# olFi95/image_search

Measured on AMD Instinct MI355X. Metric: images/sec embedded (ViT-L/14 b=256) + queries/sec cosine top-10 over 10M x 768, higher is better.
Workload: dtype bf16; 1 GPU; BASELINE config 4: per step, H2D of a pinned batch of 256 224x224x3 f32 images -> bf16 ViT-L/14 (random-init seeded weights) -> 256 rows appended to the table on the device -> cosine top-10 query over 10000000+ x 768 fp32 rows per GPU -> D2H of the k results; fused on HIP streams (the upload runs under the previous batch's tower; the scan is asynchronous to the host and runs between towers); query; batch=256, rows_per_gpu=10000000, k=10

## Files before the change

### image_search_amd/_lib.py

```python
from __future__ import annotations

import ctypes
import os

_PKG = os.path.dirname(os.path.abspath(__file__))
LIB_PATH = os.path.join(_PKG, "libmi355clip.so")

c_f = ctypes.POINTER(ctypes.c_float)
c_u64p = ctypes.POINTER(ctypes.c_uint64)
c_u8p = ctypes.POINTER(ctypes.c_uint8)
c_vp = ctypes.c_void_p

SYMBOLS = {
    "mi_last_error": (ctypes.c_char_p, []),
    "mi_abi_version": (ctypes.c_int, []),
    "mi_device_count": (ctypes.c_int, []),
    "mi_clip_load": (ctypes.c_int, [ctypes.c_char_p, ctypes.c_int, ctypes.c_int, ctypes.POINTER(c_vp)]),
    "mi_clip_free": (None, [c_vp]),
    "mi_weights_list": (ctypes.c_int, [ctypes.c_char_p, ctypes.c_char_p, ctypes.c_size_t, ctypes.POINTER(ctypes.c_size_t)]),
    "mi_clip_set_option": (ctypes.c_int, [c_vp, ctypes.c_char_p, ctypes.c_int]),
    "mi_clip_info": (ctypes.c_int, [c_vp, ctypes.POINTER(ctypes.c_uint32)]),
    "mi_clip_ln_fold_stats": (ctypes.c_int, [c_vp, ctypes.POINTER(ctypes.c_uint64), ctypes.c_int]),
    "mi_clip_embed": (ctypes.c_int, [c_vp, c_vp, ctypes.c_size_t, c_vp]),
    "mi_clip_embed_device": (ctypes.c_int, [c_vp, c_vp, ctypes.c_size_t, c_vp, c_vp]),
# ... 91 lines not shown
    "mi_pipeline_drain": (ctypes.c_int, [c_vp, ctypes.c_uint32]),
    "mi_pipeline_stats": (ctypes.c_int, [c_vp, ctypes.POINTER(ctypes.c_double), ctypes.c_int]),
    "mi_host_alloc": (ctypes.c_int, [ctypes.c_size_t, ctypes.POINTER(c_vp)]),
    "mi_host_free": (None, [c_vp]),
    "mi_average_slices": (ctypes.c_int, [ctypes.POINTER(c_f), ctypes.c_size_t, ctypes.c_size_t, c_f]),
    "mi_refine": (ctypes.c_int, [c_f, ctypes.POINTER(c_f), ctypes.c_size_t, ctypes.c_size_t, c_f]),
    "mi_op_linear": (ctypes.c_int, [ctypes.c_int, ctypes.c_int, ctypes.c_int, c_vp, c_vp, c_vp, c_vp,
                                    ctypes.c_size_t, ctypes.c_int, ctypes.c_int]),
    "mi_op_attention": (ctypes.c_int, [ctypes.c_int, ctypes.c_int, c_vp, c_vp, ctypes.c_size_t, ctypes.c_int,
                                       ctypes.c_int, ctypes.c_int]),
    "mi_op_clock_probe": (ctypes.c_int, [ctypes.c_int, c_vp, ctypes.POINTER(ctypes.c_float)]),
    "mi_op_linear_lnf": (ctypes.c_int, [ctypes.c_int, ctypes.c_int, c_vp, c_vp, c_vp, c_vp, c_vp, c_vp,
                                        ctypes.c_size_t, ctypes.c_int, ctypes.c_int]),
    "mi_op_linear_resid24": (ctypes.c_int, [ctypes.c_int, c_vp, c_vp, c_vp, c_vp, c_vp, c_vp, c_vp,
                                            ctypes.c_size_t, ctypes.c_int, ctypes.c_int, ctypes.c_float]),
    "mi_op_layernorm": (ctypes.c_int, [ctypes.c_int, ctypes.c_int, c_vp, c_vp, c_vp, c_vp, ctypes.c_size_t,
                                       ctypes.c_int, ctypes.c_float]),
}

MI_OK = 0
ERR_NAMES = {-1: "MI_ERR_INVALID", -2: "MI_ERR_IO", -3: "MI_ERR_HIP", -4: "MI_ERR_NO_DEVICE",
             -5: "MI_ERR_UNSUPPORTED", -6: "MI_ERR_OOM"}


class MiError(RuntimeError):
    def __init__(self, code: int, msg: str):
        super().__init__(f"{ERR_NAMES.get(code, code)}: {msg}")
        self.code = code


# ... 27 lines not shown
```

### image_search_amd/csrc/handles.h

```cpp
#pragma once
#include <mutex>
#include <vector>

#include "common.h"

namespace mi {
typedef unsigned short bf16_t;

struct Layer {
    float *ln1w, *ln1b, *ln2w, *ln2b;
    void *wqkv, *wo, *w1, *w2;
    float *bqkv, *bo, *b1, *b2;
    void *wqkv_f = nullptr, *w1_f = nullptr;
    float *cqkv = nullptr, *bqkv_f = nullptr, *c1 = nullptr, *b1_f = nullptr;
};


}

struct mi_clip {
    int device = 0, precision = 0;
    int image = 0, patch = 0, grid = 0, S = 0, D = 0, L = 0, H = 0, FF = 0, E = 0, Kp = 0;
    float eps = 1e-5f;
    std::vector<void*> allocs;
// ... 6 lines not shown
    float *d_in = nullptr, *d_in2 = nullptr, *d_out = nullptr, *d_out2 = nullptr;
    struct Act {
        float *patch = nullptr, *x = nullptr;
        void *col = nullptr, *y = nullptr, *qkv = nullptr, *h = nullptr;
        mi::bf16_t *delta = nullptr, *delta2 = nullptr;
        void *c_ctx = nullptr, *c_y = nullptr, *c_h = nullptr;
        float* c_x = nullptr;
        mi::bf16_t *c_d1 = nullptr, *c_d2 = nullptr;
        float *part = nullptr, *stats = nullptr;
        float* c_stats = nullptr;
    } act[4];
    hipStream_t aux[3] = {nullptr, nullptr, nullptr};
    hipEvent_t ev_fork = nullptr, ev_join[3] = {nullptr, nullptr, nullptr};
    hipEvent_t ev_embed[4] = {nullptr, nullptr, nullptr, nullptr}, ev_front[4] = {nullptr, nullptr, nullptr, nullptr};
    bool ev_embed_set[4] = {false, false, false, false};
    bool x24 = true;
    bool ln_fold = true;
    bool fold_ready = false;
    bool ln_center = true;
    unsigned long long* d_fold_offset_rows = nullptr;
    uint64_t fold_rows_checked = 0;
    int parts = 2;
    int n_cu = 256;
    uint8_t* d_rgb = nullptr;
    bool text = false;
    int vocab = 0;
    float* tok = nullptr;
    int *d_ids = nullptr, *d_rows = nullptr;
    size_t text_cap = 0;
    int* h_ids_pin = nullptr;
// ... 2 lines not shown
    hipGraph_t text_graph = nullptr;
    hipGraphExec_t text_graph_exec = nullptr;
    uint8_t* d_img_src[2] = {nullptr, nullptr};
    float* d_img_tmp = nullptr;
    size_t img_src_cap = 0, img_tmp_cap = 0;
    hipStream_t copy_stream = nullptr;
    hipEvent_t ev_up[2] = {nullptr, nullptr}, ev_used[2] = {nullptr, nullptr};
    hipStream_t stream = nullptr;
    size_t max_batch = 256;
    bool split_ln = false;
    int attn_ver = 2;
    bool q_prescaled = false;
    bool attn_shift = false;
    int qkv_pad = 128;
    int qkv_layout = 0;
    bool front_overlap = false;
    bool store_nt = true;
    bool attn_nt = false;
    int attn_order = 1;
    bool full_last = false;
    bool split_tail = true;
    int gemm_order = 4;
    bool text_fast = true;
    bool attn_f32_mfma = true;
    bool text_fuse = true;
    int ln_nt = 0;
    bool im2col_rows = true;
    mi::WorkOrder order;
    std::mutex mu;
};

// ... 145 lines not shown
```

### image_search_amd/csrc/vit.hip

```cpp
#include <algorithm>
#include <cctype>
#include <cmath>
#include <cstdio>
#include <cstring>
#include <map>
#include <mutex>
#include <string>
#include <vector>

#include "common.h"
#include "handles.h"
#include "weights.h"
#include "../../include/mi355clip_ops.h"
#include "preprocess_kernels.h"
#include "vit_kernels.h"
#include "attn32_kernels.h"

using namespace mi;

namespace {

inline uint16_t f32_to_bf16_host(float f) {
    uint32_t u;
    std::memcpy(&u, &f, 4);
    if ((u & 0x7fffffffu) > 0x7f800000u) return (uint16_t)((u >> 16) | 0x40);
    return (uint16_t)((u + 0x7fffu + ((u >> 16) & 1u)) >> 16);
}

}

namespace {
// ... 383 lines not shown
        return;
    }
    if constexpr (EPI == EPI_BIAS || EPI == EPI_BIAS_QGELU) {
        const size_t Mp = pad256(Mrows);
        if (m->precision == MI_PRECISION_BF16 && pp_shape_ok(Mp, N, K, col_stride == 64 ? ldo : N)) {
            PpFold f;
            f.col_stride = col_stride;
            launch_pp<EPI>(m, X, W, bias, out, Mp, N, K, ldo, f, s);
            return;
        }
    }
    if (col_stride != 64) fail(MI_ERR_INVALID, "head-major output needs the persistent GEMM");
    gemm_p<EPI>(m->precision, X, W, bias, out, Mrows, N, K, ldo, s);
}

#define MI_LN_DISPATCH(D, CALL)                                                              \
    switch (D) {                                                                             \
        case 128: { constexpr int VEC = 2, NT = 1; CALL; } break;                            \
        case 256: { constexpr int VEC = 4, NT = 1; CALL; } break;                            \
        case 384: { constexpr int VEC = 2, NT = 3; CALL; } break;                            \
        case 512: { constexpr int VEC = 4, NT = 2; CALL; } break;                            \
        case 768: { constexpr int VEC = 4, NT = 3; CALL; } break;                            \
        case 1024: { constexpr int VEC = 4, NT = 4; CALL; } break;                           \
        case 1280: { constexpr int VEC = 4, NT = 5; CALL; } break;                           \
        case 1536: { constexpr int VEC = 4, NT = 6; CALL; } break;                           \
        case 1664: { constexpr int VEC = 2, NT = 13; CALL; } break;                          \
        default: fail(MI_ERR_UNSUPPORTED, "hidden size %d has no LayerNorm instantiation", D); \
    }

void layer_norm(mi_clip* m, float* x, const bf16_t* d1, const bf16_t* d2, bool write_back, void* y, const float* w,
// ... 139 lines not shown
        first += np;
    }
    if (parts > 1) {
        HIP_CHECK(hipEventRecord(m->ev_fork, s0));
        for (int p = 1; p < parts; ++p) HIP_CHECK(hipStreamWaitEvent(pt[p].s, m->ev_fork, 0));
    }
    for (int p = 0; p < parts; ++p) {
        Part& q = pt[p];
        hipStream_t es_ = q.s;
        hipStream_t fs = front ? front : q.s;
        if (!m->ev_embed[p]) {
            HIP_CHECK(hipEventCreateWithFlags(&m->ev_embed[p], hipEventDisableTiming));
            HIP_CHECK(hipEventCreateWithFlags(&m->ev_front[p], hipEventDisableTiming));
        }
        if (front && m->ev_embed_set[p]) HIP_CHECK(hipStreamWaitEvent(front, m->ev_embed[p], 0));
        const size_t total = q.P * 3 * (size_t)m->patch;
        const unsigned blocks = (unsigned)std::min<size_t>((total + 255) / 256, 65535 * 4);
        if (m->precision == MI_PRECISION_F32 || is_x3(m))
            hipLaunchKernelGGL((im2col_kernel<float>), dim3(blocks), dim3(256), 0, fs, q.img, (float*)q.a->col, (int)q.n, m->grid, m->patch, m->image, m->Kp);
        else if (m->im2col_rows && m->image % 4 == 0 && (3 * m->patch * m->patch) % 4 == 0 && m->Kp % 4 == 0 && (size_t)3 * m->patch * m->image * 4 <= 64 * 1024)
            hipLaunchKernelGGL(im2col_rows_kernel, dim3((unsigned)(q.n * m->grid)), dim3(256), (size_t)3 * m->patch * m->image * 4, fs, q.img,
                               (bf16_t*)q.a->col, m->grid, m->patch, m->image, m->Kp);
        else
            hipLaunchKernelGGL((im2col_kernel<bf16_t>), dim3(blocks), dim3(256), 0, fs, q.img, (bf16_t*)q.a->col, (int)q.n, m->grid, m->patch, m->image, m->Kp);
        HIP_CHECK(hipGetLastError());
        gemm<EPI_STORE_F32>(m, q.a->col, m->wpatch, nullptr, q.a->patch, q.P, D, m->Kp, D, fs);
        if (front) {
            HIP_CHECK(hipEventRecord(m->ev_front[p], front));
            HIP_CHECK(hipStreamWaitEvent(es_, m->ev_front[p], 0));
        }
        fs = es_;
        const size_t rows_launch = fold ? pad256(q.M) : q.M;
        const unsigned lb = (unsigned)((rows_launch + 3) / 4);
        MI_LN_DISPATCH(D, hipLaunchKernelGGL((embed_ln_kernel<VEC, NT>), dim3(lb), dim3(256), 0, fs, q.a->patch, m->cls, m->pos, q.a->x, m->pre_w, m->pre_b, (int)q.M, S, m->eps, q.xlo,
                                             fold ? q.a->stats : (float*)nullptr, (int)rows_launch, fold ? m->d_fold_offset_rows : nullptr, m->ln_center ? 1 : 0));
        if (fold) m->fold_rows_checked += q.M;
        HIP_CHECK(hipEventRecord(m->ev_embed[p], fs));
        m->ev_embed_set[p] = true;
        HIP_CHECK(hipGetLastError());
    }
    const bool full_last = m->full_last;
    const int nb = D / 32;
    const int ldq = (int)qkv_pitch(m);
    const bool hm = qkv_head_major(m) && pp_shape_ok(pad256((n / parts + 1) * (size_t)S), 3 * D, D, 3 * D);
    auto hm_rows = [&](const Part& q) { return hm ? pad256(q.M) : (size_t)0; };
    auto qkv_cs = [&](const Part& q) { return hm ? (uint32_t)(pad256(q.M) * 64) : 64u; };
    const int ldq_o = hm ? 64 : ldq;
    auto ln_stats = [&](Part& q) {
        const size_t Mp = pad256(q.M);
        hipLaunchKernelGGL(ln_stats_kernel, dim3((unsigned)(Mp / 16)), dim3(256), 0, q.s, q.a->part, q.a->stats, (int)Mp, nb, 1.0f / (float)D, m->eps,
                           (int)q.M, m->d_fold_offset_rows);
        HIP_CHECK(hipGetLastError());
        m->fold_rows_checked += q.M;
    };
    for (size_t li = 0; li < m->layers.size(); ++li) {
        const Layer& ly = m->layers[li];
        const bool last = !full_last && li + 1 == m->layers.size();
// ... 20 lines not shown
                PpFold f;
                f.xlo = (uint8_t*)q.a->x + q.xlo; f.part = q.a->part;
                launch_pp<EPI_RESID24>(m, q.a->y, ly.wo, ly.bo, q.a->x, pad256(q.M), D, D, D, f, s);
                ln_stats(q);
                PpFold f1;
                f1.cvec = ly.c1; f1.stats = q.a->stats;
                launch_pp<EPI_LNF_QGELU>(m, q.a->x, ly.w1_f, ly.b1_f, q.a->h, pad256(q.M), FF, D, FF, f1, s);
                launch_pp<EPI_RESID24>(m, q.a->h, ly.w2, ly.b2, q.a->x, pad256(q.M), D, FF, D, f, s);
                ln_stats(q);
                continue;
            }
            if (last) {
                const size_t es = esize(m);
                const unsigned gb = (unsigned)std::min<size_t>((q.n * (size_t)D / 4 + 255) / 256, 4096);
                char* kv_out = (char*)q.a->qkv + (hm ? (size_t)m->H * pad256(q.M) * 64 : (size_t)D) * es;
                if (fold) {
                    PpFold f;
                    f.cvec = ly.cqkv + D; f.stats = q.a->stats; f.col_stride = qkv_cs(q);
                    launch_pp<EPI_LNF>(m, q.a->x, (const char*)ly.wqkv_f + (size_t)D * D * 2, ly.bqkv_f + D, kv_out, pad256(q.M), 2 * D, D, ldq_o, f, s);
                    hipLaunchKernelGGL((gather_rows_kernel<bf16_t>), dim3(gb), dim3(256), 0, s, (const bf16_t*)q.a->x, (bf16_t*)q.a->c_y, (int)q.n, (size_t)S, D);
                    hipLaunchKernelGGL(gather_stats_kernel, dim3((unsigned)((q.n + 255) / 256)), dim3(256), 0, s, q.a->stats, q.a->c_stats, (int)q.n, (size_t)S);
                    PpFold fq;
                    fq.cvec = ly.cqkv; fq.stats = q.a->c_stats;
                    launch_pp<EPI_LNF>(m, q.a->c_y, ly.wqkv_f, ly.bqkv_f, q.a->c_ctx, pad256(q.n), D, D, D, fq, s);
                } else {
                gemm<EPI_BIAS>(m, q.a->y, (const char*)ly.wqkv + (size_t)D * Kln * es, ly.bqkv + D, kv_out, q.M, 2 * D, Kln, ldq_o, s, qkv_cs(q));
                if (deferred) hipLaunchKernelGGL((gather_rows_kernel<bf16_t>), dim3(gb), dim3(256), 0, s, (const bf16_t*)q.a->y, (bf16_t*)q.a->c_y, (int)q.n, (size_t)S, Kln);
                else hipLaunchKernelGGL((gather_rows_kernel<float>), dim3(gb), dim3(256), 0, s, (const float*)q.a->y, (float*)q.a->c_y, (int)q.n, (size_t)S, D);
                gemm<EPI_BIAS>(m, q.a->c_y, ly.wqkv, ly.bqkv, q.a->c_ctx, q.n, D, Kln, D, s);
                }
                if (deferred) hipLaunchKernelGGL((scatter_rows_kernel<bf16_t>), dim3(gb), dim3(256), 0, s, (const bf16_t*)q.a->c_ctx, (bf16_t*)q.a->qkv, (int)q.n, (size_t)S, D, (size_t)ldq_o, (size_t)qkv_cs(q));
                else hipLaunchKernelGGL((scatter_rows_kernel<float>), dim3(gb), dim3(256), 0, s, (const float*)q.a->c_ctx, (float*)q.a->qkv, (int)q.n, (size_t)S, D, (size_t)ldq, (size_t)64);
                HIP_CHECK(hipGetLastError());
                attention(m, q.a->qkv, q.a->y, q.n, s, true, ldq, hm_rows(q));
                const unsigned gb2 = gb;
                if (deferred) hipLaunchKernelGGL((gather_rows_kernel<bf16_t>), dim3(gb2), dim3(256), 0, s, (const bf16_t*)q.a->y, (bf16_t*)q.a->c_ctx, (int)q.n, (size_t)S, D);
                else hipLaunchKernelGGL((gather_rows_kernel<float>), dim3(gb2), dim3(256), 0, s, (const float*)q.a->y, (float*)q.a->c_ctx, (int)q.n, (size_t)S, D);
                if (q.xlo) hipLaunchKernelGGL(gather_rows_x24_kernel, dim3(gb2), dim3(256), 0, s, (const uint16_t*)q.a->x, (const uint8_t*)q.a->x + q.xlo, q.a->c_x, (int)q.n, (size_t)S, D, x_bias);
                else hipLaunchKernelGGL((gather_rows_kernel<float>), dim3(gb2), dim3(256), 0, s, (const float*)q.a->x, q.a->c_x, (int)q.n, (size_t)S, D);
                HIP_CHECK(hipGetLastError());
                if (deferred) {
                    gemm<EPI_BIAS>(m, q.a->c_ctx, ly.wo, ly.bo, q.a->c_d1, q.n, D, D, D, s);
                    layer_norm(m, q.a->c_x, q.a->c_d1, nullptr, false, q.a->c_y, ly.ln2w, ly.ln2b, q.n, s);
                    gemm<EPI_BIAS_QGELU>(m, q.a->c_y, ly.w1, ly.b1, q.a->c_h, q.n, FF, Kln, FF, s);
                    gemm<EPI_BIAS>(m, q.a->c_h, ly.w2, ly.b2, q.a->c_d2, q.n, D, FF, D, s);
                } else {
                    gemm<EPI_BIAS_RESID>(m, q.a->c_ctx, ly.wo, ly.bo, q.a->c_x, q.n, D, D, D, s);
                    layer_norm(m, q.a->c_x, nullptr, nullptr, true, q.a->c_y, ly.ln2w, ly.ln2b, q.n, s);
                    gemm<EPI_BIAS_QGELU>(m, q.a->c_y, ly.w1, ly.b1, q.a->c_h, q.n, FF, Kln, FF, s);
// ... 180 lines not shown
        }
    }
    MI_LN_DISPATCH(D, hipLaunchKernelGGL((head_kernel<VEC, NT>), dim3((unsigned)((n + 7) / 8), 16), dim3(256), 0, s, a.x, p1, p2, m->post_w, m->post_b, m->proj, m->d_out, (int)n, S, m->E, m->eps, (const int*)m->d_rows));
    HIP_CHECK(hipGetLastError());
}

void free_model(mi_clip* m) {
    if (!m) return;
    (void)hipSetDevice(m->device);
    if (m->stream) { (void)hipStreamSynchronize(m->stream); (void)hipStreamDestroy(m->stream); }
    for (auto& a : m->aux) if (a) { (void)hipStreamSynchronize(a); (void)hipStreamDestroy(a); }
    m->order.destroy();
    if (m->ev_fork) (void)hipEventDestroy(m->ev_fork);
    for (auto& e : m->ev_embed) if (e) (void)hipEventDestroy(e);
    for (auto& e : m->ev_front) if (e) (void)hipEventDestroy(e);
    for (auto& e : m->ev_join) if (e) (void)hipEventDestroy(e);
    if (m->copy_stream) { (void)hipStreamSynchronize(m->copy_stream); (void)hipStreamDestroy(m->copy_stream); }
    for (int b = 0; b < 2; ++b) {
        if (m->ev_up[b]) (void)hipEventDestroy(m->ev_up[b]);
        if (m->ev_used[b]) (void)hipEventDestroy(m->ev_used[b]);
        if (m->d_img_src[b]) (void)hipFree(m->d_img_src[b]);
    }
    if (m->d_img_tmp) (void)hipFree(m->d_img_tmp);
    drop_text_graph(m);
    if (m->h_ids_pin) (void)hipHostFree(m->h_ids_pin);
    if (m->h_out_pin) (void)hipHostFree(m->h_out_pin);
    for (void* p : m->allocs) (void)hipFree(p);
    for (void* p : m->ws) (void)hipFree(p);
    delete m;
}
// ... 18 lines not shown
            const TensorInfo& t = file->info(name);
            out += name + " " + t.dtype + " [";
            for (size_t i = 0; i < t.shape.size(); ++i) out += (i ? "," : "") + std::to_string(t.shape[i]);
            out += "]\n";
        }
        for (const std::string& l : file->skipped_lines()) out += l + "\n";
        if (needed) *needed = out.size() + 1;
        if (buf && cap) {
            const size_t n = std::min(cap - 1, out.size());
            std::memcpy(buf, out.data(), n);
            buf[n] = '\0';
        }
    });
}

int mi_clip_set_option(mi_clip* m, const char* key, int value) {
    return guarded([&] {
        if (!m || !key) fail(MI_ERR_INVALID, "null argument");
        std::lock_guard<std::mutex> l(m->mu);
        DeviceGuard g(m->device);
        const std::string k(key);
        if (m->text) { m->order.sync(); drop_text_graph(m); }
        if (k == "full_last") m->full_last = value != 0;
        else if (k == "attn_shift") m->attn_shift = value != 0;
        else if (k == "front_overlap") m->front_overlap = value != 0;
        else if (k == "attn_nt") m->attn_nt = value != 0;
        else if (k == "store_nt") m->store_nt = value != 0;
        else if (k == "qkv_pad") {
            if (value < 0 || value > 1024 || value % 64) fail(MI_ERR_INVALID, "qkv_pad must be a multiple of 64 in 0..1024");
            if (m->text) fail(MI_ERR_INVALID, "the text tower's qkv rows are dense");
            if (value != m->qkv_pad) {
                m->order.sync();
                for (void* p : m->ws) HIP_CHECK(hipFree(p));
                m->ws.clear();
                m->cap = 0;
                m->qkv_pad = value;
            }
        } else if (k == "qkv_layout") {
            if (value < 0 || value > 1) fail(MI_ERR_INVALID, "qkv_layout must be 0 (token rows) or 1 (head-major planes)");
            if (m->text) fail(MI_ERR_INVALID, "the text tower's qkv rows are dense");
// ... 23 lines not shown
            m->ln_fold = value != 0;
        }
        else if (k == "max_batch") {
            if (value < 1) fail(MI_ERR_INVALID, "max_batch must be >= 1");
            m->max_batch = (size_t)value;
        } else if (k == "parts") {
            if (value < 1 || value > 4) fail(MI_ERR_INVALID, "parts must be 1..4");
            if (m->text) fail(MI_ERR_INVALID, "the text tower runs as one stream");
            if (value != m->parts) {
                m->order.sync();
                for (void* p : m->ws) HIP_CHECK(hipFree(p));
                m->ws.clear();
                m->cap = 0;
                m->parts = value;
            }
        } else fail(MI_ERR_INVALID, "unknown option '%s' (full_last, front_overlap, attn_shift, attn_nt, store_nt, attn_order, qkv_pad, qkv_layout, split_tail, gemm_order, im2col_rows, ln_nt, x24, ln_fold, text_fast, text_fuse, attn_f32_mfma, max_batch, parts)", key);
    });
}

int mi_clip_load(const char* weights_path, int device, int precision, mi_clip** out) {
    mi_clip* m = nullptr;
    const int rc = guarded([&] {
        if (!out) fail(MI_ERR_INVALID, "out is null");
        *out = nullptr;
        if (!weights_path) fail(MI_ERR_INVALID, "weights_path is null");
        if (precision != MI_PRECISION_F32 && precision != MI_PRECISION_BF16 && precision != MI_PRECISION_BF16_SPLIT &&
            precision != MI_PRECISION_BF16X3)
            fail(MI_ERR_INVALID, "precision %d: use MI_PRECISION_F32 (0), MI_PRECISION_BF16 (1), MI_PRECISION_BF16_SPLIT (2) or MI_PRECISION_BF16X3 (3)", precision);
        DeviceGuard g(device);
        m = new mi_clip();
        m->device = device;
// ... 1 lines not shown
        m->split_ln = precision == MI_PRECISION_BF16_SPLIT;
        if (const char* e = std::getenv("MI_CLIP_MAX_BATCH")) m->max_batch = std::max(1, std::atoi(e));
        HIP_CHECK(hipEventCreateWithFlags(&m->ev_fork, hipEventDisableTiming));
        for (auto& e : m->ev_join) HIP_CHECK(hipEventCreateWithFlags(&e, hipEventDisableTiming));
        if (const char* e = std::getenv("MI_CLIP_PARTS")) m->parts = std::min(4, std::max(1, std::atoi(e)));
        if (const char* e = std::getenv("MI_CLIP_FULL_LAST")) m->full_last = std::atoi(e) != 0;
        if (const char* e = std::getenv("MI_CLIP_ATTN")) m->attn_ver = std::atoi(e) == 1 ? 1 : 2;
        if (const char* e = std::getenv("MI_GEMM_SPLIT")) m->split_tail = std::atoi(e) != 0;
        if (const char* e = std::getenv("MI_GEMM_ORDER")) m->gemm_order = std::max(0, std::min(16, std::atoi(e)));
        if (const char* e = std::getenv("MI_CLIP_IM2COL")) m->im2col_rows = std::atoi(e) != 0;
        if (const char* e = std::getenv("MI_CLIP_LN_NT")) m->ln_nt = std::atoi(e) & 3;
        if (const char* e = std::getenv("MI_CLIP_X24")) m->x24 = std::atoi(e) != 0;
        if (m->precision == MI_PRECISION_BF16X3) m->x24 = false;
        if (const char* e = std::getenv("MI_CLIP_LN_CENTER")) m->ln_center = std::atoi(e) != 0;
        if (const char* e = std::getenv("MI_CLIP_QKV_LAYOUT")) m->qkv_layout = std::atoi(e) == 1 ? 1 : 0;
        if (const char* e = std::getenv("MI_CLIP_FRONT_OVERLAP")) m->front_overlap = std::atoi(e) != 0;
        hipDeviceProp_t prop;
        HIP_CHECK(hipGetDeviceProperties(&prop, device));
        m->n_cu = prop.multiProcessorCount;
        load_weights(m, weights_path);
        if (const char* e = std::getenv("MI_CLIP_LN_FOLD")) m->ln_fold = std::atoi(e) != 0 && m->fold_ready;
        *out = m;
    });
    if (rc != MI_OK && m) free_model(m);
    return rc;
}

void mi_clip_free(mi_clip* m) { free_model(m); }

int mi_clip_load_text(const char* weights_path, int device, int precision, mi_clip** out) {
    mi_clip* m = nullptr;
// ... 361 lines not shown
        void* dw = sc.up(MI_PRECISION_BF16, w, n, k, n);
        float* db = (float*)sc.up(MI_PRECISION_F32, bias, 1, n, 1);
        PpFold f;
        f.cvec = (float*)sc.up(MI_PRECISION_F32, c, 1, n, 1);
        f.stats = (float*)sc.up(MI_PRECISION_F32, stats, m_rows, 2, mp);
        void* dout = sc.bytes(mp * n * 2);
        mi_clip mm;
        op_pp_model(mm, device);
        if (epilogue == EPI_LNF) launch_pp<EPI_LNF>(&mm, dx, dw, db, dout, mp, n, k, n, f, nullptr);
        else launch_pp<EPI_LNF_QGELU>(&mm, dx, dw, db, dout, mp, n, k, n, f, nullptr);
        HIP_CHECK(hipDeviceSynchronize());
        sc.down(MI_PRECISION_BF16, dout, out, m_rows * n);
    });
}

int mi_op_linear_resid24(int device, const float* x, const float* w, const float* bias, float* xres, float* hi_out,
                         float* part, float* stats, size_t m_rows, int n, int k, float eps) {
    return guarded([&] {
        if (!x || !w || !bias || !xres) fail(MI_ERR_INVALID, "null buffer");
        const size_t mp = pad256(m_rows);
        if (!pp_shape_ok(mp, n, k, n) || mp * (size_t)(n / 32) * 8 >= (1ull << 32))
            fail(MI_ERR_UNSUPPORTED, "shape [%zu x %d x %d] is not one of the persistent GEMM's", m_rows, n, k);
        DeviceGuard g(device);
        Scratch sc;
        void* dx = sc.up(MI_PRECISION_BF16, x, m_rows, k, mp);
        void* dw = sc.up(MI_PRECISION_BF16, w, n, k, n);
        float* db = (float*)sc.up(MI_PRECISION_F32, bias, 1, n, 1);
        const size_t cnt = mp * (size_t)n;
        std::vector<uint16_t> hi(cnt, 0);
        std::vector<uint8_t> lo(cnt, 0x80);
// ... 119 lines not shown
```

### image_search_amd/ops.py

```python
from __future__ import annotations

import numpy as np

from ._lib import check, lib

EPI_STORE_F32, EPI_BIAS, EPI_BIAS_QGELU, EPI_BIAS_RESID = 0, 1, 2, 3
EPI_LNF, EPI_LNF_QGELU = 4, 5


def _f(a):
    return np.ascontiguousarray(a, np.float32)


def linear(x, w, bias=None, epilogue=EPI_BIAS, precision=0, out=None, device=0):
    x, w = _f(x), _f(w)
    m, k = x.shape
    n = w.shape[0]
    o = _f(out).copy() if out is not None else np.zeros((m, n), np.float32)
    b = _f(bias) if bias is not None else None
    check(lib().mi_op_linear(device, precision, epilogue, x.ctypes.data, w.ctypes.data,
                             b.ctypes.data if b is not None else None, o.ctypes.data, m, n, k))
    return o


# ... 22 lines not shown
                                 stats.ctypes.data, o.ctypes.data, m, n, k))
    return o


def linear_resid24(x, w, bias, xres, eps=1e-5, device=0):
    x, w, bias = _f(x), _f(w), _f(bias)
    r = _f(xres).copy()
    m, k = x.shape
    n = w.shape[0]
    hi = np.zeros((m, n), np.float32)
    part = np.zeros((m, n // 32, 2), np.float32)
    stats = np.zeros((m, 2), np.float32)
    check(lib().mi_op_linear_resid24(device, x.ctypes.data, w.ctypes.data, bias.ctypes.data, r.ctypes.data,
                                     hi.ctypes.data, part.ctypes.data, stats.ctypes.data, m, n, k, eps))
    return r, hi, part, stats
```

### include/mi355clip.h

```cpp
#ifndef MI355CLIP_H
#define MI355CLIP_H

#include <stddef.h>
#include <stdint.h>

#ifdef __cplusplus
extern "C" {
#endif

#define MI_OK 0
#define MI_ERR_INVALID (-1)
#define MI_ERR_IO (-2)
#define MI_ERR_HIP (-3)
#define MI_ERR_NO_DEVICE (-4)
#define MI_ERR_UNSUPPORTED (-5)
#define MI_ERR_OOM (-6)

#define MI_PRECISION_F32 0
#define MI_PRECISION_BF16 1
#define MI_PRECISION_BF16_SPLIT 2
#define MI_PRECISION_BF16X3 3

#define MI_KNN_NO_ID UINT64_MAX

// ... 1 lines not shown
typedef struct mi_knn mi_knn;
typedef struct mi_pipeline mi_pipeline;
typedef struct mi_knn_sharded mi_knn_sharded;
typedef struct mi_index mi_index;

const char* mi_last_error(void);
int mi_abi_version(void);
int mi_device_count(void);


int mi_clip_load(const char* weights_path, int device, int precision, mi_clip** out);
void mi_clip_free(mi_clip* m);
int mi_weights_list(const char* weights_path, char* buf, size_t cap, size_t* needed);

int mi_clip_set_option(mi_clip* m, const char* key, int value);

int mi_clip_info(const mi_clip* m, uint32_t out[8]);

int mi_clip_ln_fold_stats(mi_clip* m, uint64_t out[2], int reset);

int mi_clip_embed(mi_clip* m, const float* nchw, size_t n, float* out);

int mi_clip_embed_device(mi_clip* m, const float* d_nchw, size_t n, float* d_out, void* stream);

int mi_clip_embed_rgb8(mi_clip* m, const uint8_t* rgb8, size_t n, float* out);

int mi_preprocess_rgb8(const uint8_t* rgb8, size_t n, uint32_t height, uint32_t width, float* chw);

int mi_resize_catmullrom_rgb8(int device, const uint8_t* rgb8, uint32_t width, uint32_t height, uint32_t new_width,
                              uint32_t new_height, uint8_t* out);
// ... 120 lines not shown
```

### include/mi355clip_ops.h

```cpp
#ifndef MI355CLIP_OPS_H
#define MI355CLIP_OPS_H
#include <stddef.h>
#include <stdint.h>
#ifdef __cplusplus
extern "C" {
#endif

#define MI_EPI_STORE_F32 0
#define MI_EPI_BIAS 1
#define MI_EPI_BIAS_QGELU 2
#define MI_EPI_BIAS_RESID 3

int mi_op_linear(int device, int precision, int epilogue, const float* x, const float* w, const float* bias,
                 float* out, size_t m_rows, int n, int k);

#define MI_EPI_LNF 4
#define MI_EPI_LNF_QGELU 5
int mi_op_linear_lnf(int device, int epilogue, const float* x, const float* w, const float* bias, const float* c,
                     const float* stats, float* out, size_t m_rows, int n, int k);
int mi_op_linear_resid24(int device, const float* x, const float* w, const float* bias, float* xres, float* hi_out,
                         float* part, float* stats, size_t m_rows, int n, int k, float eps);

int mi_op_attention(int device, int precision, const float* qkv, float* ctx, size_t n_img, int s_tok, int d,
                    int heads);

int mi_op_layernorm(int device, int precision, const float* x, const float* w, const float* b, float* y,
                    size_t rows, int d, float eps);

int mi_op_clock_probe(int device, void* stream, float* mhz);

#ifdef __cplusplus
}
#endif
#endif
```

Baseline: 6628 images/s.

## Add dedicated CLS-row tail kernels for the last layer and overlap next front

Adds a CLS tail path, on by default, for the deferred last layer. Only the CLS rows get their Q projection, out-projection, LN2 and MLP, through a small MFMA GEMM kernel that reads strided CLS rows directly, which removes the gather and scatter kernels and the generic GEMM launches that are inefficient at tiny M. A fused LN2 kernel reads the packed residual in place. A new front_overlap=2 mode lets the next batch's front end wait only on the tail event after attention rather than on the full embed. It also adds option validation and a test entry point. The cost is more code paths, and the new GEMM streams weights without LDS reuse.

```diff
diff --git a/image_search_amd/_lib.py b/image_search_amd/_lib.py
--- a/image_search_amd/_lib.py
+++ b/image_search_amd/_lib.py
@@ -129,6 +129,9 @@
                                         ctypes.c_size_t, ctypes.c_int, ctypes.c_int]),
     "mi_op_linear_resid24": (ctypes.c_int, [ctypes.c_int, c_vp, c_vp, c_vp, c_vp, c_vp, c_vp, c_vp,
                                             ctypes.c_size_t, ctypes.c_int, ctypes.c_int, ctypes.c_float]),
+    "mi_clip_option_check": (ctypes.c_int, [ctypes.c_char_p, ctypes.c_int]),
+    "mi_op_linear_cls": (ctypes.c_int, [ctypes.c_int, ctypes.c_int, c_vp, c_vp, c_vp, c_vp, c_vp, c_vp,
+                                        ctypes.c_size_t, ctypes.c_int, ctypes.c_int, ctypes.c_size_t, ctypes.c_int]),
     "mi_op_layernorm": (ctypes.c_int, [ctypes.c_int, ctypes.c_int, c_vp, c_vp, c_vp, c_vp, ctypes.c_size_t,
                                        ctypes.c_int, ctypes.c_float]),
 }
diff --git a/image_search_amd/csrc/cls_tail_kernels.h b/image_search_amd/csrc/cls_tail_kernels.h
--- /dev/null
+++ b/image_search_amd/csrc/cls_tail_kernels.h
@@ -0,0 +1,95 @@
+#pragma once
+#include "vit_kernels.h"
+
+namespace mi {
+
+constexpr int CLS_ROWS = 64;
+
+template <int EPI, int P>
+__global__ __launch_bounds__(256) void cls_gemm_kernel(const bf16_t* __restrict__ X, size_t ldx, const bf16_t* __restrict__ W, int K,
+                                                       const float* __restrict__ bias, const float* __restrict__ cvec,
+                                                       const float* __restrict__ stats, size_t ld_stats, bf16_t* __restrict__ out,
+                                                       size_t ldo, uint32_t cs, int M) {
+    static_assert(EPI == EPI_BIAS || EPI == EPI_BIAS_QGELU || EPI == EPI_LNF, "the tail's three epilogues");
+    const int lane = threadIdx.x & 63, wave = threadIdx.x >> 6, g = lane >> 4, l15 = lane & 15;
+    const int n0 = blockIdx.x * 16;
+    const int m0 = blockIdx.y * CLS_ROWS + wave * 16;
+    if (m0 >= M) return;
+    const int row = min(m0 + l15, M - 1);
+    const bf16_t* wp = W + (size_t)(n0 + l15) * K + 8 * g;
+    const bf16_t* xp = X + (size_t)row * ldx + 8 * g;
+    bf16x8 a[P], b[P];
+#pragma unroll
+    for (int i = 0; i < P; ++i) {
+        a[i] = *reinterpret_cast<const bf16x8*>(wp + 32 * i);
+        b[i] = *reinterpret_cast<const bf16x8*>(xp + 32 * i);
+    }
+    const v4f b4 = *reinterpret_cast<const v4f*>(bias + n0 + 4 * g);
+    v4f c4 = (v4f){0.0f, 0.0f, 0.0f, 0.0f};
+    v2f st = (v2f){0.0f, 0.0f};
+    if constexpr (EPI == EPI_LNF) {
+        c4 = *reinterpret_cast<const v4f*>(cvec + n0 + 4 * g);
+        st = *reinterpret_cast<const v2f*>(stats + (size_t)row * ld_stats * 2);
+    }
+    v4f acc = (v4f){0.0f, 0.0f, 0.0f, 0.0f};
+    const int steps = K / 32;
+    for (int k = P; k < steps; k += P) {
+#pragma unroll
+        for (int i = 0; i < P; ++i) {
+            acc = __builtin_amdgcn_mfma_f32_16x16x32_bf16(a[i], b[i], acc, 0, 0, 0);
+            a[i] = *reinterpret_cast<const bf16x8*>(wp + 32 * (k + i));
+            b[i] = *reinterpret_cast<const bf16x8*>(xp + 32 * (k + i));
+        }
+    }
+#pragma unroll
+    for (int i = 0; i < P; ++i) acc = __builtin_amdgcn_mfma_f32_16x16x32_bf16(a[i], b[i], acc, 0, 0, 0);
+    v4f v;
+    if constexpr (EPI == EPI_LNF) {
+#pragma unroll
+        for (int c = 0; c < 4; ++c) v[c] = __builtin_fmaf(st.x, acc[c], __builtin_fmaf(st.y, c4[c], b4[c]));
+    } else {
+        v = acc + b4;
+    }
+    if constexpr (EPI == EPI_BIAS_QGELU) {
+#pragma unroll
+        for (int c = 0; c < 4; ++c) v[c] = quick_gelu<true>(v[c]);
+    }
+    if (m0 + l15 >= M) return;
+    const int col = n0 + 4 * g;
+    v2u pk;
+    pk.x = pack2bf(v[0], v[1]);
+    pk.y = pack2bf(v[2], v[3]);
+    *reinterpret_cast<v2u*>(out + (size_t)row * ldo + (size_t)(col >> 6) * cs + (col & 63)) = pk;
+}
+
+template <int VEC, int NT>
+__global__ __launch_bounds__(256) void cls_ln2_kernel(const float* __restrict__ x, size_t x_lo_off, uint32_t x_bias, size_t S,
+                                                      const bf16_t* __restrict__ d1, float* __restrict__ cx, bf16_t* __restrict__ y,
+                                                      const float* __restrict__ w, const float* __restrict__ b, int rows, float eps,
+                                                      int y_ld, int split) {
+    constexpr int D = 64 * VEC * NT;
+    const int lane = threadIdx.x & 63;
+    const int row = blockIdx.x * 4 + (threadIdx.x >> 6);
+    if (row >= rows) return;
+    const size_t src = (size_t)row * S * D;
+    LnRow<VEC, NT> r;
+    bool packed = false;
+    if constexpr (VEC == 4) {
+        if (x_lo_off) {
+            r.load_x24(reinterpret_cast<const uint16_t*>(x) + src, reinterpret_cast<const uint8_t*>(x) + x_lo_off + src, lane, x_bias);
+            packed = true;
+        }
+    }
+    if (!packed) r.load(x + src, lane);
+    r.store(cx + (size_t)row * D, lane);
+    r.add_bf16(d1 + (size_t)row * D, lane);
+    r.normalize(w, b, eps, lane);
+    r.store(y + (size_t)row * y_ld, lane);
+    if (split) {
+#pragma unroll
+        for (int j = 0; j < VEC * NT; ++j) r.v[j] -= bf2f(f2bf(r.v[j]));
+        r.store(y + (size_t)row * y_ld + D, lane);
+    }
+}
+
+}
diff --git a/image_search_amd/csrc/handles.h b/image_search_amd/csrc/handles.h
--- a/image_search_amd/csrc/handles.h
+++ b/image_search_amd/csrc/handles.h
@@ -44,6 +44,8 @@
     hipEvent_t ev_fork = nullptr, ev_join[3] = {nullptr, nullptr, nullptr};
     hipEvent_t ev_embed[4] = {nullptr, nullptr, nullptr, nullptr}, ev_front[4] = {nullptr, nullptr, nullptr, nullptr};
     bool ev_embed_set[4] = {false, false, false, false};
+    hipEvent_t ev_tail[4] = {nullptr, nullptr, nullptr, nullptr};
+    bool ev_tail_set[4] = {false, false, false, false};
     bool x24 = true;
     bool ln_fold = true;
     bool fold_ready = false;
@@ -76,7 +78,8 @@
     bool attn_shift = false;
     int qkv_pad = 128;
     int qkv_layout = 0;
-    bool front_overlap = false;
+    bool cls_tail = true;
+    int front_overlap = 0;
     bool store_nt = true;
     bool attn_nt = false;
     int attn_order = 1;
diff --git a/image_search_amd/csrc/vit.hip b/image_search_amd/csrc/vit.hip
--- a/image_search_amd/csrc/vit.hip
+++ b/image_search_amd/csrc/vit.hip
@@ -15,6 +15,7 @@
 #include "preprocess_kernels.h"
 #include "vit_kernels.h"
 #include "attn32_kernels.h"
+#include "cls_tail_kernels.h"
 
 using namespace mi;
 
@@ -428,6 +429,22 @@
     gemm_p<EPI>(m->precision, X, W, bias, out, Mrows, N, K, ldo, s);
 }
 
+bool cls_gemm_shape_ok(int N, int K) { return N % 16 == 0 && K % 256 == 0; }
+template <int EPI>
+void launch_cls_gemm(const void* X, size_t ldx, const void* W, const float* bias, const float* cvec, const float* stats, size_t ld_stats,
+                     void* out, size_t ldo, uint32_t cs, size_t M, int N, int K, hipStream_t s) {
+    if (M == 0) return;
+    if (!cls_gemm_shape_ok(N, K)) fail(MI_ERR_UNSUPPORTED, "CLS GEMM: N=%d must be a multiple of 16 and K=%d of 256", N, K);
+    const dim3 grid((unsigned)(N / 16), (unsigned)((M + CLS_ROWS - 1) / CLS_ROWS));
+    if (K % 512 == 0)
+        hipLaunchKernelGGL((cls_gemm_kernel<EPI, 16>), grid, dim3(256), 0, s, (const bf16_t*)X, ldx, (const bf16_t*)W, K, bias, cvec, stats, ld_stats,
+                           (bf16_t*)out, ldo, cs, (int)M);
+    else
+        hipLaunchKernelGGL((cls_gemm_kernel<EPI, 8>), grid, dim3(256), 0, s, (const bf16_t*)X, ldx, (const bf16_t*)W, K, bias, cvec, stats, ld_stats,
+                           (bf16_t*)out, ldo, cs, (int)M);
+    HIP_CHECK(hipGetLastError());
+}
+
 #define MI_LN_DISPATCH(D, CALL)                                                              \
     switch (D) {                                                                             \
         case 128: { constexpr int VEC = 2, NT = 1; CALL; } break;                            \
@@ -597,6 +614,9 @@
             HIP_CHECK(hipEventCreateWithFlags(&m->ev_front[p], hipEventDisableTiming));
         }
         if (front && m->ev_embed_set[p]) HIP_CHECK(hipStreamWaitEvent(front, m->ev_embed[p], 0));
+        if (front && p == 0 && m->front_overlap == 2)
+            for (int t = 0; t < 4; ++t)
+                if (m->ev_tail_set[t]) HIP_CHECK(hipStreamWaitEvent(front, m->ev_tail[t], 0));
         const size_t total = q.P * 3 * (size_t)m->patch;
         const unsigned blocks = (unsigned)std::min<size_t>((total + 255) / 256, 65535 * 4);
         if (m->precision == MI_PRECISION_F32 || is_x3(m))
@@ -624,6 +644,10 @@
     }
     const bool full_last = m->full_last;
     const int nb = D / 32;
+    const size_t np_max = pad256(n / parts + 1);
+    const bool cls_tail = m->cls_tail && deferred && cls_gemm_shape_ok(D, fold ? D : Kln) && cls_gemm_shape_ok(D, D) &&
+                          cls_gemm_shape_ok(FF, Kln) && cls_gemm_shape_ok(D, FF) && pp_shape_ok(np_max, D, fold ? D : Kln, D) &&
+                          pp_shape_ok(np_max, D, D, D) && pp_shape_ok(np_max, FF, Kln, FF) && pp_shape_ok(np_max, D, FF, D);
     const int ldq = (int)qkv_pitch(m);
     const bool hm = qkv_head_major(m) && pp_shape_ok(pad256((n / parts + 1) * (size_t)S), 3 * D, D, 3 * D);
     auto hm_rows = [&](const Part& q) { return hm ? pad256(q.M) : (size_t)0; };
@@ -674,6 +698,33 @@
                 const size_t es = esize(m);
                 const unsigned gb = (unsigned)std::min<size_t>((q.n * (size_t)D / 4 + 255) / 256, 4096);
                 char* kv_out = (char*)q.a->qkv + (hm ? (size_t)m->H * pad256(q.M) * 64 : (size_t)D) * es;
+                if (cls_tail) {
+                    const size_t ldo_q = (size_t)S * ldq_o;
+                    if (fold) {
+                        launch_cls_gemm<EPI_LNF>(q.a->x, (size_t)S * D, ly.wqkv_f, ly.bqkv_f, ly.cqkv, q.a->stats, (size_t)S, q.a->qkv, ldo_q, qkv_cs(q),
+                                                 q.n, D, D, s);
+                        PpFold f;
+                        f.cvec = ly.cqkv + D; f.stats = q.a->stats; f.col_stride = qkv_cs(q);
+                        launch_pp<EPI_LNF>(m, q.a->x, (const char*)ly.wqkv_f + (size_t)D * D * 2, ly.bqkv_f + D, kv_out, pad256(q.M), 2 * D, D, ldq_o, f, s);
+                    } else {
+                        launch_cls_gemm<EPI_BIAS>(q.a->y, (size_t)S * Kln, ly.wqkv, ly.bqkv, nullptr, nullptr, 0, q.a->qkv, ldo_q, qkv_cs(q), q.n, D, Kln, s);
+                        gemm<EPI_BIAS>(m, q.a->y, (const char*)ly.wqkv + (size_t)D * Kln * es, ly.bqkv + D, kv_out, q.M, 2 * D, Kln, ldq_o, s, qkv_cs(q));
+                    }
+                    attention(m, q.a->qkv, q.a->y, q.n, s, true, ldq, hm_rows(q));
+                    if (!m->ev_tail[p]) HIP_CHECK(hipEventCreateWithFlags(&m->ev_tail[p], hipEventDisableTiming));
+                    HIP_CHECK(hipEventRecord(m->ev_tail[p], s));
+                    m->ev_tail_set[p] = true;
+                    launch_cls_gemm<EPI_BIAS>(q.a->y, (size_t)S * D, ly.wo, ly.bo, nullptr, nullptr, 0, q.a->c_d1, D, 64, q.n, D, D, s);
+                    MI_LN_DISPATCH(D, hipLaunchKernelGGL((cls_ln2_kernel<VEC, NT>), dim3((unsigned)((q.n + 3) / 4)), dim3(256), 0, s, q.a->x, q.xlo, x_bias, (size_t)S,
+                                                         q.a->c_d1, q.a->c_x, (bf16_t*)q.a->c_y, ly.ln2w, ly.ln2b, (int)q.n, m->eps, Kln, m->split_ln ? 1 : 0));
+                    HIP_CHECK(hipGetLastError());
+                    launch_cls_gemm<EPI_BIAS_QGELU>(q.a->c_y, Kln, ly.w1, ly.b1, nullptr, nullptr, 0, q.a->c_h, FF, 64, q.n, FF, Kln, s);
+                    launch_cls_gemm<EPI_BIAS>(q.a->c_h, FF, ly.w2, ly.b2, nullptr, nullptr, 0, q.a->c_d2, D, 64, q.n, D, FF, s);
+                    const unsigned hy = (unsigned)std::max(16, std::min(64, m->E / 16));
+                    MI_LN_DISPATCH(D, hipLaunchKernelGGL((head_kernel<VEC, NT>), dim3((unsigned)((q.n + 7) / 8), hy), dim3(256), 0, s, q.a->c_x, q.a->c_d1, q.a->c_d2, m->post_w, m->post_b, m->proj, q.out, (int)q.n, 1, m->E, m->eps, (const int*)nullptr));
+                    HIP_CHECK(hipGetLastError());
+                    continue;
+                }
                 if (fold) {
                     PpFold f;
                     f.cvec = ly.cqkv + D; f.stats = q.a->stats; f.col_stride = qkv_cs(q);
@@ -693,6 +744,9 @@
                 else hipLaunchKernelGGL((scatter_rows_kernel<float>), dim3(gb), dim3(256), 0, s, (const float*)q.a->c_ctx, (float*)q.a->qkv, (int)q.n, (size_t)S, D, (size_t)ldq, (size_t)64);
                 HIP_CHECK(hipGetLastError());
                 attention(m, q.a->qkv, q.a->y, q.n, s, true, ldq, hm_rows(q));
+                if (!m->ev_tail[p]) HIP_CHECK(hipEventCreateWithFlags(&m->ev_tail[p], hipEventDisableTiming));
+                HIP_CHECK(hipEventRecord(m->ev_tail[p], s));
+                m->ev_tail_set[p] = true;
                 const unsigned gb2 = gb;
                 if (deferred) hipLaunchKernelGGL((gather_rows_kernel<bf16_t>), dim3(gb2), dim3(256), 0, s, (const bf16_t*)q.a->y, (bf16_t*)q.a->c_ctx, (int)q.n, (size_t)S, D);
                 else hipLaunchKernelGGL((gather_rows_kernel<float>), dim3(gb2), dim3(256), 0, s, (const float*)q.a->y, (float*)q.a->c_ctx, (int)q.n, (size_t)S, D);
@@ -903,6 +957,7 @@
     if (m->ev_fork) (void)hipEventDestroy(m->ev_fork);
     for (auto& e : m->ev_embed) if (e) (void)hipEventDestroy(e);
     for (auto& e : m->ev_front) if (e) (void)hipEventDestroy(e);
+    for (auto& e : m->ev_tail) if (e) (void)hipEventDestroy(e);
     for (auto& e : m->ev_join) if (e) (void)hipEventDestroy(e);
     if (m->copy_stream) { (void)hipStreamSynchronize(m->copy_stream); (void)hipStreamDestroy(m->copy_stream); }
     for (int b = 0; b < 2; ++b) {
@@ -951,16 +1006,61 @@
     });
 }
 
+namespace {
+struct OptionSpec { const char* key; int lo, hi; const char* bounds; };
+constexpr int OPT_MIN = -2147483647 - 1, OPT_MAX = 2147483647;
+const OptionSpec kOptions[] = {
+    {"full_last", OPT_MIN, OPT_MAX, ""},
+    {"front_overlap", 0, 2, "front_overlap must be 0 (off), 1 (behind the upload) or 2 (under the previous forward's CLS tail)"},
+    {"cls_tail", OPT_MIN, OPT_MAX, ""},
+    {"attn_shift", OPT_MIN, OPT_MAX, ""},
+    {"attn_nt", OPT_MIN, OPT_MAX, ""},
+    {"store_nt", OPT_MIN, OPT_MAX, ""},
+    {"attn_order", 0, 1, "attn_order must be 0 or 1"},
+    {"qkv_pad", 0, 1024, "qkv_pad must be a multiple of 64 in 0..1024"},
+    {"qkv_layout", 0, 1, "qkv_layout must be 0 (token rows) or 1 (head-major planes)"},
+    {"split_tail", OPT_MIN, OPT_MAX, ""},
+    {"gemm_order", 0, 16, "gemm_order must be 0..16"},
+    {"im2col_rows", OPT_MIN, OPT_MAX, ""},
+    {"ln_nt", OPT_MIN, OPT_MAX, ""},
+    {"x24", OPT_MIN, OPT_MAX, ""},
+    {"ln_fold", OPT_MIN, OPT_MAX, ""},
+    {"text_fast", OPT_MIN, OPT_MAX, ""},
+    {"text_fuse", OPT_MIN, OPT_MAX, ""},
+    {"attn_f32_mfma", OPT_MIN, OPT_MAX, ""},
+    {"max_batch", 1, OPT_MAX, "max_batch must be >= 1"},
+    {"parts", 1, 4, "parts must be 1..4"},
+};
+void option_check(const char* key, int value) {
+    if (!key) fail(MI_ERR_INVALID, "null argument");
+    std::string names;
+    for (const OptionSpec& o : kOptions) {
+        if (std::strcmp(o.key, key) == 0) {
+            if (value < o.lo || value > o.hi) fail(MI_ERR_INVALID, "%s", o.bounds);
+            return;
+        }
+        names += (names.empty() ? "" : ", ") + std::string(o.key);
+    }
+    fail(MI_ERR_INVALID, "unknown option '%s' (%s)", key, names.c_str());
+}
+}
+
+int mi_clip_option_check(const char* key, int value) {
+    return guarded([&] { option_check(key, value); });
+}
+
 int mi_clip_set_option(mi_clip* m, const char* key, int value) {
     return guarded([&] {
         if (!m || !key) fail(MI_ERR_INVALID, "null argument");
+        option_check(key, value);
         std::lock_guard<std::mutex> l(m->mu);
         DeviceGuard g(m->device);
         const std::string k(key);
         if (m->text) { m->order.sync(); drop_text_graph(m); }
         if (k == "full_last") m->full_last = value != 0;
         else if (k == "attn_shift") m->attn_shift = value != 0;
-        else if (k == "front_overlap") m->front_overlap = value != 0;
+        else if (k == "front_overlap") m->front_overlap = value;
+        else if (k == "cls_tail") m->cls_tail = value != 0;
         else if (k == "attn_nt") m->attn_nt = value != 0;
         else if (k == "store_nt") m->store_nt = value != 0;
         else if (k == "qkv_pad") {
@@ -1014,7 +1114,7 @@
                 m->cap = 0;
                 m->parts = value;
             }
-        } else fail(MI_ERR_INVALID, "unknown option '%s' (full_last, front_overlap, attn_shift, attn_nt, store_nt, attn_order, qkv_pad, qkv_layout, split_tail, gemm_order, im2col_rows, ln_nt, x24, ln_fold, text_fast, text_fuse, attn_f32_mfma, max_batch, parts)", key);
+        } else fail(MI_ERR_INVALID, "option '%s' is listed but not handled", key);
     });
 }
 
@@ -1046,7 +1146,8 @@
         if (m->precision == MI_PRECISION_BF16X3) m->x24 = false;
         if (const char* e = std::getenv("MI_CLIP_LN_CENTER")) m->ln_center = std::atoi(e) != 0;
         if (const char* e = std::getenv("MI_CLIP_QKV_LAYOUT")) m->qkv_layout = std::atoi(e) == 1 ? 1 : 0;
-        if (const char* e = std::getenv("MI_CLIP_FRONT_OVERLAP")) m->front_overlap = std::atoi(e) != 0;
+        if (const char* e = std::getenv("MI_CLIP_FRONT_OVERLAP")) m->front_overlap = std::max(0, std::min(2, std::atoi(e)));
+        if (const char* e = std::getenv("MI_CLIP_CLS_TAIL")) m->cls_tail = std::atoi(e) != 0;
         hipDeviceProp_t prop;
         HIP_CHECK(hipGetDeviceProperties(&prop, device));
         m->n_cu = prop.multiProcessorCount;
@@ -1438,6 +1539,45 @@
     });
 }
 
+int mi_op_linear_cls(int device, int epilogue, const float* x, const float* w, const float* bias, const float* c, const float* stats,
+                     float* out, size_t m_rows, int n, int k, size_t row_stride, int head_major) {
+    return guarded([&] {
+        if (!x || !w || !bias || !out) fail(MI_ERR_INVALID, "null buffer");
+        if (epilogue != EPI_BIAS && epilogue != EPI_BIAS_QGELU && epilogue != EPI_LNF) fail(MI_ERR_INVALID, "epilogue %d (EPI_BIAS, EPI_BIAS_QGELU or EPI_LNF)", epilogue);
+        if (epilogue == EPI_LNF && (!c || !stats)) fail(MI_ERR_INVALID, "EPI_LNF needs c and stats");
+        if (m_rows == 0 || row_stride == 0) fail(MI_ERR_INVALID, "m_rows and row_stride must be positive");
+        if (!cls_gemm_shape_ok(n, k) || (head_major && n % 64)) fail(MI_ERR_UNSUPPORTED, "shape [%zu x %d x %d] is not one of the CLS GEMM's", m_rows, n, k);
+        DeviceGuard g(device);
+        Scratch sc;
+        const size_t rows = (m_rows - 1) * row_stride + 1;
+        std::vector<uint16_t> hx(rows * (size_t)k, 0x7FC1), ho(rows * (size_t)n, 0xFFFF);
+        std::vector<float> hs(rows * 2, std::nanf(""));
+        for (size_t r = 0; r < m_rows; ++r) {
+            for (size_t j = 0; j < (size_t)k; ++j) hx[r * row_stride * k + j] = f32_to_bf16_host(x[r * k + j]);
+            if (stats) { hs[r * row_stride * 2] = stats[r * 2]; hs[r * row_stride * 2 + 1] = stats[r * 2 + 1]; }
+        }
+        void* dx = sc.bytes(hx.size() * 2);
+        void* dout = sc.bytes(ho.size() * 2);
+        float* ds = (float*)sc.bytes(hs.size() * 4);
+        HIP_CHECK(hipMemcpy(dx, hx.data(), hx.size() * 2, hipMemcpyHostToDevice));
+        HIP_CHECK(hipMemcpy(dout, ho.data(), ho.size() * 2, hipMemcpyHostToDevice));
+        HIP_CHECK(hipMemcpy(ds, hs.data(), hs.size() * 4, hipMemcpyHostToDevice));
+        void* dw = sc.up(MI_PRECISION_BF16, w, n, k, n);
+        float* db = (float*)sc.up(MI_PRECISION_F32, bias, 1, n, 1);
+        float* dc = c ? (float*)sc.up(MI_PRECISION_F32, c, 1, n, 1) : nullptr;
+        const size_t ldo = row_stride * (head_major ? (size_t)64 : (size_t)n);
+        const uint32_t cs = head_major ? (uint32_t)(rows * 64) : 64u;
+        if (head_major && rows * 64 >= (1ull << 32)) fail(MI_ERR_UNSUPPORTED, "head-major planes of %zu rows", rows);
+        switch (epilogue) {
+            case EPI_BIAS: launch_cls_gemm<EPI_BIAS>(dx, row_stride * k, dw, db, nullptr, nullptr, 0, dout, ldo, cs, m_rows, n, k, nullptr); break;
+            case EPI_BIAS_QGELU: launch_cls_gemm<EPI_BIAS_QGELU>(dx, row_stride * k, dw, db, nullptr, nullptr, 0, dout, ldo, cs, m_rows, n, k, nullptr); break;
+            default: launch_cls_gemm<EPI_LNF>(dx, row_stride * k, dw, db, dc, ds, row_stride, dout, ldo, cs, m_rows, n, k, nullptr); break;
+        }
+        HIP_CHECK(hipDeviceSynchronize());
+        sc.down(MI_PRECISION_BF16, dout, out, rows * (size_t)n);
+    });
+}
+
 int mi_op_linear_resid24(int device, const float* x, const float* w, const float* bias, float* xres, float* hi_out,
                          float* part, float* stats, size_t m_rows, int n, int k, float eps) {
     return guarded([&] {
diff --git a/image_search_amd/ops.py b/image_search_amd/ops.py
--- a/image_search_amd/ops.py
+++ b/image_search_amd/ops.py
@@ -60,3 +60,17 @@
     check(lib().mi_op_linear_resid24(device, x.ctypes.data, w.ctypes.data, bias.ctypes.data, r.ctypes.data,
                                      hi.ctypes.data, part.ctypes.data, stats.ctypes.data, m, n, k, eps))
     return r, hi, part, stats
+
+
+def linear_cls(x, w, bias, c=None, stats=None, epilogue=EPI_BIAS, row_stride=1, head_major=False, device=0):
+    x, w, bias = _f(x), _f(w), _f(bias)
+    c = _f(c) if c is not None else None
+    stats = _f(stats) if stats is not None else None
+    m, k = x.shape
+    n = w.shape[0]
+    rows = (m - 1) * row_stride + 1
+    o = np.zeros((n // 64, rows, 64) if head_major else (rows, n), np.float32)
+    check(lib().mi_op_linear_cls(device, epilogue, x.ctypes.data, w.ctypes.data, bias.ctypes.data,
+                                 c.ctypes.data if c is not None else None, stats.ctypes.data if stats is not None else None,
+                                 o.ctypes.data, m, n, k, row_stride, 1 if head_major else 0))
+    return (o.view(np.uint32) >> 16).astype(np.uint16)
diff --git a/include/mi355clip.h b/include/mi355clip.h
--- a/include/mi355clip.h
+++ b/include/mi355clip.h
@@ -39,6 +39,7 @@
 int mi_weights_list(const char* weights_path, char* buf, size_t cap, size_t* needed);
 
 int mi_clip_set_option(mi_clip* m, const char* key, int value);
+int mi_clip_option_check(const char* key, int value);
 
 int mi_clip_info(const mi_clip* m, uint32_t out[8]);
 
diff --git a/include/mi355clip_ops.h b/include/mi355clip_ops.h
--- a/include/mi355clip_ops.h
+++ b/include/mi355clip_ops.h
@@ -21,6 +21,9 @@
 int mi_op_linear_resid24(int device, const float* x, const float* w, const float* bias, float* xres, float* hi_out,
                          float* part, float* stats, size_t m_rows, int n, int k, float eps);
 
+int mi_op_linear_cls(int device, int epilogue, const float* x, const float* w, const float* bias, const float* c, const float* stats,
+                     float* out, size_t m_rows, int n, int k, size_t row_stride, int head_major);
+
 int mi_op_attention(int device, int precision, const float* qkv, float* ctx, size_t n_img, int s_tok, int d,
                     int heads);
 
```

New measurement: 6633 images/s, median of 2. No clear change (+0.1%).
